# kaleo996/F5E-TTS

Measured on AMD Instinct MI355X. Metric: mel_frames_per_sec, higher is better.
Workload: dtype bf16; 1 GPU; C2: F5TTS_v1_Base random-init, batch 1 per GPU, N_ref=188 N=469 frames, euler NFE=32, CFG=2.0 (cond+uncond batched), sway=-1.0, hipGraph ODE loop, HIP log-mel front-end + Vocos decode on GPU; parallelism=replica x1 (utterance sharding, no collective on the data path)

## Files before the change

f5e-tts_amd/_C.py:

```python
from __future__ import annotations

import ctypes as C
import os

_HERE = os.path.dirname(os.path.abspath(__file__))
LIB_PATH = os.environ.get("F5E_HIP_LIB") or os.path.join(_HERE, "libf5e_hip.so")

ABI_VERSION = 2

ACT_NONE, ACT_SILU, ACT_GELU_ERF, ACT_GELU_TANH, ACT_RELU, ACT_MISH = range(6)

_P, _I, _F, _LL = C.c_void_p, C.c_int, C.c_float, C.c_longlong

SIGNATURES = {
    "f5e_abi_version": [],
    "f5e_last_error": [],
    "f5e_check_device": [],
    "f5e_gemm_bf16_bias": [_P, _P, _I, _P, _I, _P, _P, _I, _I, _I, _I, _I, _I, _I],
    "f5e_gemm_bf16_gate_residual": [_P, _P, _I, _P, _I, _P, _P, _I, _P, _I, _I, _P, _I, _I, _P, _I, _I, _I, _I],
    "f5e_gemm_bf16_qkv_rope": [_P, _P, _I, _P, _I, _P, _P, _P, _P, _I, _I, _I, _P, _P, _P, _I, _I, _I, _I],
    "f5e_gemm_bf16_bias_ln": [_P, _P, _I, _P, _I, _P, _P, _I, _I, _I, _I, _I, _I, _I, _P],
    "f5e_gemm_bf16_gate_residual_ln": [_P, _P, _I, _P, _I, _P, _P, _I, _P, _I, _I, _P, _I, _I, _P, _I, _I, _I, _I, _P],
    "f5e_gemm_bf16_qkv_rope_ln": [_P, _P, _I, _P, _I, _P, _P, _P, _P, _I, _I, _I, _P, _P, _P, _I, _I, _I, _I, _P],
    "f5e_adaln_pre": [_P, _P, _I, _P, _I, _P, _I, _I, _I, _P, _I, _P, _I, _P, _I, _I],
    "f5e_flash_attn": [_P, _P, _P, _P, _P, _I, _P, _I, _I, _I, _I, _I],
    "f5e_joint_attn": [_P, _P, _P, _P, _P, _P, _P, _P, _I, _P, _I, _P, _I, _I, _I, _I, _I, _I, _I],
    "f5e_layernorm": [_P, _P, _I, _P, _I, _I, _P, _P, _P, _P, _I, _I, _I, _P, _I, _I, _I, _F],
    "f5e_grn": [_P, _P, _P, _P, _P, _P, _I, _I, _I],
    "f5e_l2norm": [_P, _P, _I, _P, _I, _I, _P, _I, _I],
    "f5e_gemm_f32": [_P, _P, _I, _I, _I, _P, _I, _P, _I, _P, _P, _I, _I, _P, _P, _I, _P, _I, _I, _I, _I],
    "f5e_convpos": [_P, _P, _I, _P, _P, _I, _P, _I, _P, _I, _P, _I, _I, _I, _I, _I],
    "f5e_dwconv7": [_P, _P, _P, _P, _P, _I, _I, _I],
    "f5e_im2col": [_P, _P, _P, _I, _I, _I, _I, _I],
    "f5e_conv2d_sub_f32": [_P, _P, _P, _P, _P, _I, _I, _I, _I, _I, _I, _I, _I],
    "f5e_sinus_embed": [_P, _P, _P, _P, _I, _I, _F],
    "f5e_rope_table": [_P, _P, _P, _I, _I],
    "f5e_text_gather": [_P, _P, _P, _P, _P, _P, _I, _I, _I, _I, _I],
    "f5e_ode_update": [_P, _P, _LL, _I, _F, _F, _P, _P, _P, _P, _P, _P, _LL],
    "f5e_ode_update_traj": [_P, _P, _LL, _I, _F, _F, _P, _P, _P, _LL, _I, _P, _P, _P, _LL],
    "f5e_advance_eval": [_P, _P],
    "f5e_stitch": [_P, _P, _P, _P, _P, _LL, _I],
    "f5e_cast_bf16": [_P, _P, _P, _LL],
    "f5e_cast_f32": [_P, _P, _P, _LL],
    "f5e_axpby": [_P, _P, _P, _P, _F, _F, _F, _LL],
    "f5e_vq_eval": [_P, _P, _I, _P, _I, _P, _P, _P, _I, _I, _I, _I],
    "f5e_mas_workspace_bytes": [_I, _I, _I, C.POINTER(C.c_ulonglong)],
    "f5e_mas_path": [_P, _P, _LL, _I, _P, _P, _P, _P, _P, C.c_ulonglong, _I, _I, _I],
    "f5e_resample": [_P, _P, _LL, _P, _I, _I, _I, _P, _LL, _I, _I, _I],
    "f5e_ctc_align_workspace_bytes": [_I, _I, _I, C.POINTER(C.c_ulonglong)],
    "f5e_ctc_align": [_P, _P, _LL, _I, _P, _I, _P, _P, _I, _P, _P, _P, _P, _P, C.c_ulonglong, _I, _I, _I, _I],
    "f5e_ctc_greedy": [_P, _P, _LL, _I, _P, _I, _I, _P, _P, _P, _I, _I, _I],
    "f5e_ctc_loss_workspace_bytes": [_I, _I, C.POINTER(C.c_ulonglong)],
# ... 131 lines not shown
```

f5e-tts_amd/csrc/elementwise.hip:

```cpp
#include "f5e_common.h"

namespace {

inline int grid_for(size_t total) {
  size_t g = (total + 255) / 256;
  return (int)(g < 2048 ? (g ? g : 1) : 2048);
}

__global__ void sinus_embed_kernel(const float* t, const float* freqs, float* out, int E, int dim, float scale) {
  const int half = dim / 2;
  const int i = blockIdx.x * blockDim.x + threadIdx.x;
  if (i >= E * half) return;
  const int e = i / half, k = i - e * half;
  const float arg = (scale * t[e]) * freqs[k];
  float s, c;
  sincosf(arg, &s, &c);
  out[(size_t)e * dim + k] = s;
  out[(size_t)e * dim + half + k] = c;
}

__global__ void rope_table_kernel(const float* inv_freq, float* out, int N, int half) {
  const int i = blockIdx.x * blockDim.x + threadIdx.x;
  if (i >= N * half) return;
  const int n = i / half, k = i - n * half;
// ... 6 lines not shown

__global__ void text_gather_kernel(const int* ids, const float* table, const float* pos, const float* keep, float* out,
                                   int B, int N, int TD, int max_pos, int table_rows) {
  const int td4 = TD / 4;
  const size_t total = (size_t)B * N * td4;
  for (size_t i = (size_t)blockIdx.x * 256 + threadIdx.x; i < total; i += (size_t)gridDim.x * 256) {
    const int c = (int)(i % td4) * 4;
    const size_t bn = i / td4;
    const int n = (int)(bn % N);
    const int id = min(max(ids[bn], 0), table_rows - 1);
    f32x4 v = *(const f32x4*)(table + (size_t)id * TD + c);
    if (pos) v += *(const f32x4*)(pos + (size_t)min(n, max_pos - 1) * TD + c);
    if (keep) v *= keep[bn];
    *(f32x4*)(out + bn * TD + c) = v;
  }
}

__global__ void ode_update_kernel(const float* pred, size_t branch_stride, int mode, float w0, float w1,
                                  const float* base, float* dst, float* traj, size_t traj_stride, int traj_div,
                                  const float* coef, int* eval_ptr, unsigned* done_ctr, size_t n) {
  const int e = eval_ptr ? load_uniform_i32(eval_ptr) : 0;
  const float h = __builtin_bit_cast(float, load_uniform_i32((const int*)(coef + e)));
  if (traj && traj_stride) traj += (size_t)((e + 1) / traj_div) * traj_stride;
  for (size_t i = (size_t)blockIdx.x * 256 + threadIdx.x; i < n; i += (size_t)gridDim.x * 256) {
    const float p0 = pred[i];
    float v = p0;
    if (mode == 1) {
      v = p0 + (p0 - pred[i + branch_stride]) * w0;
    } else if (mode == 2) {
      const float p1 = pred[i + branch_stride], p2 = pred[i + 2 * branch_stride];
// ... 122 lines not shown
  const int total = N * half;
  hipLaunchKernelGGL(rope_table_kernel, dim3((total + 255) / 256), dim3(256), 0, st, inv_freq, out, N, half);
  F5E_LAUNCH_CHECK("rope_table");
  return F5E_OK;
}

int f5e_text_gather(hipStream_t st, const int* ids, const float* table, const float* pos, const float* keep,
                    float* out, int B, int N, int TD, int max_pos, int table_rows) {
  F5E_REQUIRE(ids && table && out && B > 0 && N > 0 && TD > 0 && TD % 4 == 0 && table_rows > 0, "text_gather: bad arguments");
  hipLaunchKernelGGL(text_gather_kernel, dim3(grid_for((size_t)B * N * TD / 4)), dim3(256), 0, st, ids, table, pos,
                     keep, out, B, N, TD, max_pos, table_rows);
  F5E_LAUNCH_CHECK("text_gather");
  return F5E_OK;
}

int f5e_ode_update(hipStream_t st, const float* pred, long long branch_stride, int mode, float w0, float w1,
                   const float* base, float* dst, float* traj, const float* coef, int* eval_ptr, unsigned* done_ctr,
                   long long n) {
  return f5e_ode_update_traj(st, pred, branch_stride, mode, w0, w1, base, dst, traj, 0, 1, coef, eval_ptr, done_ctr, n);
}

int f5e_ode_update_traj(hipStream_t st, const float* pred, long long branch_stride, int mode, float w0, float w1,
                        const float* base, float* dst, float* traj, long long traj_stride, int traj_div,
                        const float* coef, int* eval_ptr, unsigned* done_ctr, long long n) {
  F5E_REQUIRE(pred && base && dst && coef && n > 0, "ode_update: bad arguments");
  F5E_REQUIRE(mode >= 0 && mode <= 2, "ode_update: mode must be 0 (plain), 1 (cfg) or 2 (three-branch)");
  F5E_REQUIRE(!done_ctr || eval_ptr, "ode_update: done_ctr (auto-advance) needs eval_ptr");
  F5E_REQUIRE(traj_stride >= 0 && traj_div >= 1 && (traj_stride == 0 || eval_ptr), "ode_update: bad trajectory indexing");
  hipLaunchKernelGGL(ode_update_kernel, dim3(grid_for((size_t)n)), dim3(256), 0, st, pred, (size_t)branch_stride, mode,
                     w0, w1, base, dst, traj, (size_t)traj_stride, traj_div, coef, eval_ptr, done_ctr, (size_t)n);
// ... 60 lines not shown
```

f5e-tts_amd/csrc/gemm_f32.hip:

```cpp
#include "f5e_common.h"

namespace {

struct Gemm32Args {
  const float* A; int lda; int a_rows; int a_act;
  const float* W; int ldw;
  const float* bias;
  int act;
  const float* ch_scale;
  const float* addend; int ld_add; int add_rows;
  const float* row_scale;
  float* out; int ldo;
  bf16* out_bf16; int ldo_bf16;
  int M, N, K;
  int tiles_m;
  int vec;
};

__global__ __launch_bounds__(256) void gemm_f32_kernel(Gemm32Args a) {
  constexpr int BK = 16, LDS_ROW = 17;
  __shared__ float As[2][64 * LDS_ROW];
  __shared__ float Ws[2][64 * LDS_ROW];
  const int tid = threadIdx.x, lane = tid & 63, wave = tid >> 6;
  const int tile_n = blockIdx.x / a.tiles_m, tile_m = blockIdx.x - tile_n * a.tiles_m;
// ... 267 lines not shown
                            int add_rows, const float* row_scale, float* out, int ldo, void* out_bf16, int ldo_bf16,
                            int M, int N, int K) {
  F5E_REQUIRE(A && W && (out || out_bf16), "gemm_f32: null operand");
  F5E_REQUIRE(M > 0 && N > 0 && K > 0, "gemm_f32: empty problem M=%d N=%d K=%d", M, N, K);
  F5E_REQUIRE(K % 4 == 0 && lda % 4 == 0 && ldw % 4 == 0, "gemm_f32: K, lda, ldw must be multiples of 4 (K=%d)", K);
  F5E_REQUIRE(a_rows > 0, "gemm_f32: a_rows must be positive");
  if (addend) F5E_REQUIRE(add_rows > 0, "gemm_f32: add_rows must be positive");
  Gemm32Args a{};
  a.A = A; a.lda = lda; a.a_rows = a_rows; a.a_act = a_act; a.W = W; a.ldw = ldw; a.bias = bias; a.act = act;
  a.ch_scale = ch_scale; a.addend = addend; a.ld_add = ld_add; a.add_rows = add_rows > 0 ? add_rows : 1;
  a.row_scale = row_scale; a.out = out; a.ldo = ldo; a.out_bf16 = (bf16*)out_bf16; a.ldo_bf16 = ldo_bf16;
  a.M = M; a.N = N; a.K = K;
  a.vec = N % 4 == 0 && N >= 4 && ldo % 4 == 0 && ldo_bf16 % 4 == 0 && ld_add % 4 == 0 &&
          (((uintptr_t)bias | (uintptr_t)ch_scale | (uintptr_t)addend | (uintptr_t)out) & 15) == 0 && ((uintptr_t)out_bf16 & 7) == 0;
  if (a_act == F5E_ACT_NONE && (((uintptr_t)A | (uintptr_t)W) & 15) == 0) {
    if (((M + 63) / 64) * ((N + 63) / 64) < 128) return launch_dma<32, 64, 2, 2, 4>(a, st);
    return launch_dma<64, 64, 2, 2, 3>(a, st);
  }
  a.tiles_m = (M + 63) / 64;
  const int grid = a.tiles_m * ((N + 63) / 64);
  hipLaunchKernelGGL(gemm_f32_kernel, dim3(grid), dim3(256), 0, st, a);
  F5E_LAUNCH_CHECK("gemm_f32");
  return F5E_OK;
}
```

f5e-tts_amd/csrc/norm.hip:

```cpp
#include "f5e_common.h"

namespace {

struct LnArgs {
  const float* x; int ldx;
  void* y; int ldy; int y_bf16;
  const float* gamma; const float* beta;
  const float* scale; const float* shift;
  int mod_stride, mod_rows, rows_per_seq;
  int rows, D;
  float eps;
  const int* eval_ptr; int eval_stride;
};

template <int VPL>
__global__ __launch_bounds__(256) void layernorm_kernel(LnArgs a) {
  const int lane = threadIdx.x & 63;
  const int row = blockIdx.x * 4 + (threadIdx.x >> 6);
  if (row >= a.rows) return;
  const float* xp = a.x + (size_t)row * a.ldx;
  f32x4 v[VPL];
#pragma unroll
  for (int i = 0; i < VPL; ++i) v[i] = *(const f32x4*)(xp + (i * 64 + lane) * 4);
  const int mrow = a.scale ? (row / a.rows_per_seq) % a.mod_rows : 0;
// ... 50 lines not shown
#pragma unroll
  for (int i = 0; i < 8; ++i)
    if (i * 64 + lane < nv) {
      v[i] -= mean;
      ss += (v[i][0] * v[i][0] + v[i][1] * v[i][1]) + (v[i][2] * v[i][2] + v[i][3] * v[i][3]);
    }
  const float rstd = rsqrtf(wave_sum(ss) / (float)a.D + a.eps);
#pragma unroll
  for (int i = 0; i < 8; ++i) {
    const int c = (i * 64 + lane) * 4;
    if (c < a.D) {
      f32x4 y = v[i] * rstd;
      if (a.gamma) y = y * *(const f32x4*)(a.gamma + c) + *(const f32x4*)(a.beta + c);
      *(f32x4*)((float*)a.y + (size_t)row * a.ldy + c) = y;
    }
  }
}

template <int VPL>
__global__ __launch_bounds__(256) void adaln_pre_kernel(const float* x, int ldx, bf16* xs, int ld_xs, const float* scale,
                                                        int mod_stride, int mod_rows, int rows_per_seq,
                                                        const int* eval_ptr, int eval_stride, float* stats, int parts,
                                                        float* row_mean, int rows, int D) {
  const int lane = threadIdx.x & 63;
  const int row = blockIdx.x * 4 + (threadIdx.x >> 6);
  if (row >= rows) return;
  const float* xp = x + (size_t)row * ldx;
  f32x4 v[VPL], sc[VPL];
#pragma unroll
  for (int i = 0; i < VPL; ++i) v[i] = *(const f32x4*)(xp + (i * 64 + lane) * 4);
// ... 154 lines not shown
  F5E_REQUIRE(D % 256 == 0 && D >= 256 && D <= 2048, "layernorm: D=%d must be a multiple of 256 in [256, 2048]", D);
  switch (D / 256) {
    case 1: hipLaunchKernelGGL(layernorm_kernel<1>, grid, block, 0, st, a); break;
    case 2: hipLaunchKernelGGL(layernorm_kernel<2>, grid, block, 0, st, a); break;
    case 3: hipLaunchKernelGGL(layernorm_kernel<3>, grid, block, 0, st, a); break;
    case 4: hipLaunchKernelGGL(layernorm_kernel<4>, grid, block, 0, st, a); break;
    case 5: hipLaunchKernelGGL(layernorm_kernel<5>, grid, block, 0, st, a); break;
    case 6: hipLaunchKernelGGL(layernorm_kernel<6>, grid, block, 0, st, a); break;
    case 7: hipLaunchKernelGGL(layernorm_kernel<7>, grid, block, 0, st, a); break;
    default: hipLaunchKernelGGL(layernorm_kernel<8>, grid, block, 0, st, a); break;
  }
  F5E_LAUNCH_CHECK("layernorm");
  return F5E_OK;
}

int f5e_adaln_pre(hipStream_t st, const float* x, int ldx, void* xs, int ld_xs, const float* scale, int mod_stride,
                  int mod_rows, int rows_per_seq, const int* eval_ptr, int eval_stride, float* stats, int parts,
                  float* row_mean, int rows, int D) {
  F5E_REQUIRE(x && xs && scale && stats && row_mean && rows > 0, "adaln_pre: null/empty");
  F5E_REQUIRE(D % 256 == 0 && D >= 256 && D <= 2048, "adaln_pre: D=%d must be a multiple of 256 in [256, 2048]", D);
  F5E_REQUIRE(ldx % 4 == 0 && ld_xs % 4 == 0 && mod_stride % 4 == 0, "adaln_pre: strides must be multiples of 4");
  F5E_REQUIRE(parts > 0 && parts <= 32 && mod_rows > 0 && rows_per_seq > 0, "adaln_pre: bad parts / modulation rows");
  const dim3 grid((rows + 3) / 4), block(256);
#define F5E_PRE_CASE(V)                                                                                               \
  case V: hipLaunchKernelGGL(adaln_pre_kernel<V>, grid, block, 0, st, x, ldx, (bf16*)xs, ld_xs, scale, mod_stride,    \
                             mod_rows, rows_per_seq, eval_ptr, eval_stride, stats, parts, row_mean, rows, D); break;
  switch (D / 256) {
    F5E_PRE_CASE(1) F5E_PRE_CASE(2) F5E_PRE_CASE(3) F5E_PRE_CASE(4) F5E_PRE_CASE(5) F5E_PRE_CASE(6) F5E_PRE_CASE(7)
    default: hipLaunchKernelGGL(adaln_pre_kernel<8>, grid, block, 0, st, x, ldx, (bf16*)xs, ld_xs, scale, mod_stride,
                                mod_rows, rows_per_seq, eval_ptr, eval_stride, stats, parts, row_mean, rows, D); break;
// ... 42 lines not shown
```

f5e-tts_amd/engine.py:

```python
from __future__ import annotations

import math
import os
import threading
from dataclasses import dataclass
from typing import Dict, List, Optional, Tuple

import torch

from . import _C, ops

Tensor = torch.Tensor
BF, F32, I32 = torch.bfloat16, torch.float32, torch.int32


@dataclass
class DiTConfig:
    dim: int = 1024
    depth: int = 22
    heads: int = 16
    dim_head: int = 64
    ff_mult: int = 2
    mel_dim: int = 100
    text_num_embeds: int = 2545
# ... 234 lines not shown
        temb = self.time_embed(t2.reshape(-1))
        mod = torch.empty(E * rows, self.row_stride, device=dv)
        D = cfg.dim
        for l, (w, b) in enumerate(self.adaln):
            ops.gemm_f32(temb, w, b, out=mod[:, l * 6 * D:(l + 1) * 6 * D], a_act=ops.ACT_SILU)
        ops.gemm_f32(temb, self.final_w, self.final_b, out=mod[:, self.L * 6 * D:], a_act=ops.ACT_SILU)
        self._last_temb = temb
        return mod.view(E, rows, self.row_stride)

    def text_embed(self, text: Optional[Tensor], B: int, N: int, drop_text: bool) -> Tensor:
        return self.text_embed_multi(text, B, N, (drop_text,))[0]

    def text_embed_multi(self, text: Optional[Tensor], B: int, N: int, drops: Tuple[bool, ...]) -> List[Tensor]:
        cfg, dv = self.cfg, self.device
        V = len(drops)
        keep = None
        if text is None:
            ids = torch.zeros(V * B, N, dtype=I32, device=dv)
        else:
            if text.device.type == "cpu" and text[:, :N].numel():
                hi, lo = int(text[:, :N].max()), int(text[:, :N].min())
                if hi + 1 >= self.text_table.shape[0] or lo < -1:
                    raise IndexError(f"index out of range in self: token id {hi if hi + 1 >= self.text_table.shape[0] else lo} "
                                     f"with text_num_embeds = {self.text_table.shape[0] - 1}")
            ids = (h2d(text, dv) + 1)[:, :N]
            ids = torch.nn.functional.pad(ids, (0, N - ids.shape[1]), value=0)
            if cfg.text_mask_padding:
                keep = (ids != 0).to(F32).repeat(V, 1).contiguous()
            ids = torch.cat([torch.zeros_like(ids) if d else ids for d in drops], 0).to(I32).contiguous()
        TD = cfg.text_dim
        VB = V * B
        h = torch.empty(VB, N, TD, device=dv)
        ops.text_gather(ids, self.text_table, self.text_pos, keep if self.text_blocks else None, h)
        if self.text_blocks:
            c = torch.empty_like(h)
            n = torch.empty_like(h)
            p1 = torch.empty(VB, N, 2 * TD, device=dv)
            g = torch.empty_like(p1)
            gws = torch.empty(VB, 2 * TD, device=dv)
            keep_flat = keep.view(-1) if keep is not None else None
            for blk in self.text_blocks:
                ops.dwconv7(h, blk["dw_w"], blk["dw_b"], c)
                ops.layernorm(c.view(VB * N, TD), n.view(VB * N, TD), gamma=blk["ln_g"], beta=blk["ln_b"])
                ops.gemm_f32(n.view(VB * N, TD), blk["w1"], blk["b1"], out=p1.view(VB * N, 2 * TD), act=ops.ACT_GELU_ERF)
                ops.grn(p1, g, blk["grn_g"], blk["grn_b"], gws)
                h_new = torch.empty_like(h)
                ops.gemm_f32(g.view(VB * N, 2 * TD), blk["w2"], blk["b2"], out=h_new.view(VB * N, TD),
                             addend=h.view(VB * N, TD), row_scale=keep_flat)
                h = h_new
        return [h[v * B:(v + 1) * B] for v in range(V)]

    def ppg_embed(self, ppg: Optional[Tensor], B: int, N: int, drop_ppg: bool) -> Tensor:
        cfg, dv, P = self.cfg, self.device, self.ppg
        pd = cfg.ppg_dim
        x = torch.zeros(B, N, pd, device=dv)
        if ppg is not None and not drop_ppg:
            x[:, : ppg.shape[1]] = ppg.to(dv, F32)[:, :N]
        if cfg.ppg_transformer:
# ... 371 lines not shown
    cache: Dict[tuple, Tensor] = {}
    drops = tuple(sorted({dt_ for _, dt_, _ in inp.branches}))
    for dt_, emb in zip(drops, engine.text_embed_multi(inp.text, B, N, drops)):
        cache[("t", dt_)] = emb
    for bi, (da, dt_, dp) in enumerate(inp.branches):
        tk = ("t", dt_)
        pe = None
        if cfg.use_ppg:
            pk = ("p", dp)
            if pk not in cache:
                cache[pk] = engine.ppg_embed(inp.ppg, B, N, dp)
            pe = cache[pk]
        engine.input_const(inp.step_cond, cache[tk], pe, da, in_const[bi * B * N:(bi + 1) * B * N])
    if masked:
        seq_len.copy_(setup["seq_len"].repeat(nb))
    bf["ctr"].zero_()
    y.copy_(inp.y0)
    traj[0].copy_(inp.y0)

    if fresh:
        def plans_for(y_in, first_ws):
            out = []
            for c in range(n_chains):
                lo, hi = c * per * B * N, (c + 1) * per * B * N
                sl = seq_len[c * per * B:(c + 1) * per * B] if seq_len is not None else None
                out.append(engine.make_plan(per * B, B, N, y_in, in_const[lo:hi], mod, eval_ptr, rope_cs, sl,
                                            pred=pred_all[lo:hi], cd=cd, arena=bf["ws"][first_ws + c]))
            return out

        st.plans_a = plans_for(y, 0)
        st.plans_b = plans_for(y_mid, n_chains) if y_mid is not None else None
    if st.pool is None or st.pool.owner is not st:
        for pl in st.plans_a + (st.plans_b or []):
# ... 97 lines not shown
```

f5e-tts_amd/model/cfm.py:

```python
from __future__ import annotations

from typing import Callable, NamedTuple, Optional

import torch
import torch.nn.functional as F
from torch import nn

from .. import _C
from ..engine import SamplerInputs, h2d, ode_setup, run_ode
from .modules import MelSpec
from .utils import default, exists, intersperse, lens_to_mask, list_str_to_idx, list_str_to_tensor

F32, I32 = torch.float32, torch.int32


class Alignment(NamedTuple):
    token_of_frame: torch.Tensor
    durations: torch.Tensor
    text_len: torch.Tensor
    ppg_len: torch.Tensor


class CFM(nn.Module):
    def __init__(self, transformer: nn.Module, sigma=0.0, odeint_kwargs: dict = dict(method="euler"),
                 audio_drop_prob=0.3, cond_drop_prob=0.2, num_channels=None, mel_spec_module: nn.Module | None = None,
                 mel_spec_kwargs: dict = dict(), frac_lengths_mask: tuple[float, float] = (0.7, 1.0),
                 vocab_char_map: dict[str, int] | None = None, ppg_config=dict(use_ppg=False),
                 cb_config=dict(use_codebook=False)):
        super().__init__()
        self.frac_lengths_mask = frac_lengths_mask
        self.mel_spec = default(mel_spec_module, MelSpec(**mel_spec_kwargs))
        self.num_channels = default(num_channels, self.mel_spec.n_mel_channels)
        self.audio_drop_prob, self.cond_drop_prob = audio_drop_prob, cond_drop_prob
        self.transformer = transformer
        self.dim = transformer.dim
# ... 56 lines not shown
        else:
            dur_h = torch.maximum(lens_h + 1, dur_h)
        dur_h = dur_h.clamp(max=max_duration)
        n = int(dur_h.amax())
        test_cond = None
        if duplicate_test:
            test_cond = F.pad(cond, (0, 0, cond_seq_len, n - 2 * cond_seq_len), value=0.0)
        cond = F.pad(cond, (0, 0, 0, n - cond_seq_len), value=0.0)
        if no_ref_audio:
            cond = torch.zeros_like(cond)
        if edit_mask is not None:
            cond_mask = h2d(cond_mask, dv) & edit_mask.to(dv)
        cond_mask = h2d(F.pad(cond_mask, (0, n - cond_mask.shape[-1]), value=False), dv).unsqueeze(-1)
        from .. import ops
        cond = cond.contiguous()
        step_cond = ops.stitch(cond, torch.zeros_like(cond), cond_mask.reshape(-1).to(torch.uint8).contiguous(),
                               torch.empty_like(cond))
        seq_len = dur_h.to(I32) if batch > 1 else None
        y0 = torch.zeros(batch, n, self.num_channels, dtype=F32)
        for i, dur in enumerate(dur_h.tolist()):
            if exists(seed):
                gen = torch.Generator().manual_seed(seed)
                y0[i, :dur] = torch.randn(dur, self.num_channels, dtype=F32, generator=gen)
            else:
                y0[i, :dur] = torch.randn(dur, self.num_channels, dtype=F32)
        y0 = h2d(y0, dv)
        t_start = 0
        if duplicate_test:
            t_start = t_inter
            y0 = ops.axpby(y0, test_cond.contiguous(), torch.empty_like(y0), 1 - t_start, t_start)
            steps = int(steps * (1 - t_start))
# ... 6 lines not shown
        eng = self.transformer.engine()
        inp = SamplerInputs(step_cond=prep["step_cond"], text=prep["text"], ppg=ppg, y0=prep["y0"], t=prep["t"],
                            seq_len=prep["seq_len"], branches=branches, mode=mode, w0=w0, w1=w1,
                            method=self.odeint_kwargs.get("method", "euler"))
        if self.use_graph:
            side = getattr(self._tls, "stream", None)
            if side is None:
                side = self._tls.stream = torch.cuda.Stream(device=eng.device)
            setup = ode_setup(eng, inp)
            trajectory = run_ode(eng, inp, use_graph=True, chains=self.chains, setup=setup, capture_stream=side)
        else:
            trajectory = run_ode(eng, inp, use_graph=False, timer=self.kernel_timer, chains=self.chains)
        self.transformer.clear_cache()
        out = torch.empty_like(trajectory[-1])
        from .. import ops
        ops.stitch(prep["cond"].contiguous(), trajectory[-1], prep["cond_mask"].reshape(-1).to(torch.uint8).contiguous(),
                   out)
        if exists(vocoder):
            out = vocoder(out.permute(0, 2, 1))
        return out, trajectory


    @torch.no_grad()
    def sample(self, cond, text, ppg=None, duration=None, *, lens=None, steps=32, cfg_strength=1.0,
               sway_sampling_coef=None, seed: Optional[int] = None, max_duration=4096,
               vocoder: Optional[Callable] = None, no_ref_audio=False, duplicate_test=False, t_inter=0.1,
               edit_mask=None):
        prep = self._prepare(cond, text, duration, lens, steps, sway_sampling_coef, seed, max_duration, no_ref_audio,
                             duplicate_test, t_inter, edit_mask, use_text=True)
        if cfg_strength < 1e-5:
            return self._integrate(prep, ppg, [(False, False, False)], 0, 0.0, 0.0, vocoder)
# ... 55 lines not shown
```

f5e-tts_amd/ops.py:

```python
from __future__ import annotations

import ctypes as C
import threading
from typing import Optional

import torch

from . import _C
from ._C import ACT_GELU_ERF, ACT_GELU_TANH, ACT_MISH, ACT_NONE, ACT_RELU, ACT_SILU, check, lib

Tensor = torch.Tensor
_checked_device = False


def _stream() -> int:
    return torch.cuda.current_stream().cuda_stream


def require_device() -> None:
    global _checked_device
    if not _checked_device:
        if not torch.cuda.is_available():
            raise _C.F5EError("f5e_tts_amd needs a ROCm GPU (gfx950); torch.cuda.is_available() is False and there "
                              "is no CPU fallback")
# ... 246 lines not shown
                            mode, _p(out_bf16, BF, "out_bf16"), out_bf16.stride(0) if out_bf16 is not None else 0,
                            _p(out_f32, F32, "out_f32"), out_f32.stride(0) if out_f32 is not None else 0,
                            _p(resid, F32, "resid"), resid.stride(0) if resid is not None else 0, S, N, D,
                            w_packed.shape[0]),
          "f5e_convpos")


def dwconv7(x: Tensor, w_t: Tensor, bias: Tensor, out: Tensor):
    require_device()
    B, T, Cc = x.shape
    check(lib().f5e_dwconv7(_stream(), _p(x, F32, "x"), _p(w_t, F32, "w_t"), _p(bias, F32, "bias"), _p(out, F32, "out"),
                            B, T, Cc), "f5e_dwconv7")
    return out


def im2col(x: Tensor, col: Tensor, ksize: int, pad: int):
    require_device()
    B, T, Cin = x.shape
    check(lib().f5e_im2col(_stream(), _p(x, F32, "x"), _p(col, F32, "col"), B, T, Cin, ksize, pad), "f5e_im2col")
    return col


def pack_conv2d_sub_weight(w: Tensor) -> Tensor:
    return w.permute(0, 2, 3, 1).contiguous()


def conv2d_sub(x: Tensor, w_packed: Tensor, bias: Optional[Tensor], stride: int, *, out: Optional[Tensor] = None,
               act: int = ACT_RELU) -> Tensor:
    require_device()
    if x.ndim != 4 or w_packed.ndim != 4:
# ... 26 lines not shown

def rope_table(inv_freq: Tensor, out: Tensor):
    require_device()
    N, half, _ = out.shape
    check(lib().f5e_rope_table(_stream(), _p(inv_freq, F32, "inv_freq"), _p(out, F32, "out"), N, half), "f5e_rope_table")
    return out


def text_gather(ids: Tensor, table: Tensor, pos: Optional[Tensor], keep: Optional[Tensor], out: Tensor):
    require_device()
    B, N, TD = out.shape
    check(lib().f5e_text_gather(_stream(), _p(ids, I32, "ids"), _p(table, F32, "table"), _p(pos, F32, "pos"),
                                _p(keep, F32, "keep"), _p(out, F32, "out"), B, N, TD,
                                pos.shape[0] if pos is not None else 1, table.shape[0]), "f5e_text_gather")
    return out


def ode_update(pred: Tensor, branch_stride: int, mode: int, w0: float, w1: float, base: Tensor, dst: Tensor,
               coef: Tensor, eval_ptr: Optional[Tensor], traj: Optional[Tensor] = None,
               done_ctr: Optional[Tensor] = None, traj_stride: int = 0, traj_div: int = 1):
    require_device()
    check(lib().f5e_ode_update_traj(_stream(), _p(pred, F32, "pred"), branch_stride, mode, w0, w1, _p(base, F32, "base"),
                                    _p(dst, F32, "dst"), C.c_void_p(traj.data_ptr()) if traj is not None else None,
                                    traj_stride, traj_div, _p(coef, F32, "coef"), _p(eval_ptr, I32, "eval_ptr"),
                                    _p(done_ctr, I32, "done_ctr"), base.numel()), "f5e_ode_update")
    return dst


def sample_loop(loop: "_C.LoopPlan"):
    require_device()
# ... 974 lines not shown
```

f5e-tts_amd/vocoder.py:

```python
from __future__ import annotations

import os
from typing import Optional

import torch
from torch import nn

from . import _C, ops
from .engine import fft_tables

F32 = torch.float32


class _ConvNeXtBlock(nn.Module):
    def __init__(self, dim, intermediate_dim, layer_scale_init_value):
        super().__init__()
        self.dwconv = nn.Conv1d(dim, dim, kernel_size=7, padding=3, groups=dim)
        self.norm = nn.LayerNorm(dim, eps=1e-6)
        self.pwconv1 = nn.Linear(dim, intermediate_dim)
        self.act = nn.GELU()
        self.pwconv2 = nn.Linear(intermediate_dim, dim)
        self.gamma = nn.Parameter(layer_scale_init_value * torch.ones(dim))


# ... 69 lines not shown
            raise _C.F5EError("Vocos.decode expects [b, n_mels, t]")
        dv = mel.device
        w = self._pack(dv)
        B, Cin, T = mel.shape
        if T < 2:
            raise _C.F5EError("Vocos.decode needs at least 2 frames")
        x = mel.to(F32).transpose(1, 2).contiguous()
        dim = w["embed_b"].shape[0]
        col = torch.empty(B, T, 7 * Cin, device=dv)
        ops.im2col(x, col, 7, 3)
        h = torch.empty(B * T, dim, device=dv)
        ops.gemm_f32(col.view(B * T, 7 * Cin), w["embed_w"], w["embed_b"], out=h)
        hn = torch.empty_like(h)
        ops.layernorm(h, hn, gamma=w["norm_g"], beta=w["norm_b"])
        h = hn
        c = torch.empty_like(h)
        n = torch.empty_like(h)
        inter = w["blocks"][0]["w1"].shape[0] if w["blocks"] else dim
        p1 = torch.empty(B * T, inter, device=dv)
        for blk in w["blocks"]:
            ops.dwconv7(h.view(B, T, dim), blk["dw_w"], blk["dw_b"], c.view(B, T, dim))
            ops.layernorm(c, n, gamma=blk["ln_g"], beta=blk["ln_b"])
            ops.gemm_f32(n, blk["w1"], blk["b1"], out=p1, act=ops.ACT_GELU_ERF)
            h_new = torch.empty_like(h)
            ops.gemm_f32(p1, blk["w2"], blk["b2"], out=h_new, ch_scale=blk["gamma"], addend=h)
            h = h_new
        ops.layernorm(h, n, gamma=w["fin_g"], beta=w["fin_b"])
        n_fft, hop = self.head.n_fft, self.head.hop_length
        z = torch.empty(B * T, n_fft + 2, device=dv)
        ops.gemm_f32(n, w["out_w"], w["out_b"], out=z)
        frames = torch.empty(B * T, n_fft, device=dv)
        wav = torch.empty(B, hop * (T - 1), device=dv)
        ops.istft_head(z, w["window"], w["twiddle"], frames, wav, B, T, n_fft, hop)
        return wav

    def forward(self, mel):
        return self.decode(mel)
# ... 11 lines not shown
```

include/f5e_abi.h:

```cpp
#ifndef F5E_ABI_H_
#define F5E_ABI_H_

#ifdef __cplusplus
extern "C" {
#endif

#define F5E_ABI_VERSION 2

#if defined(__GNUC__)
#define F5E_API __attribute__((visibility("default")))
#else
#define F5E_API
#endif

enum { F5E_OK = 0, F5E_ERR_BAD_SHAPE = -1, F5E_ERR_UNSUPPORTED = -2, F5E_ERR_HIP = -3 };

enum { F5E_ACT_NONE = 0, F5E_ACT_SILU = 1, F5E_ACT_GELU_ERF = 2, F5E_ACT_GELU_TANH = 3, F5E_ACT_RELU = 4, F5E_ACT_MISH = 5 };

#ifdef F5E_STREAM_T
typedef F5E_STREAM_T f5e_stream;
#else
typedef void* f5e_stream;
#endif

// ... 57 lines not shown
F5E_API int f5e_grn(f5e_stream st, const float* x, float* y, float* gx_ws, const float* gamma, const float* beta, int B, int T,
            int C);


F5E_API int f5e_gemm_f32(f5e_stream st, const float* A, int lda, int a_rows, int a_act, const float* W, int ldw,
                 const float* bias, int act, const float* ch_scale, const float* addend, int ld_add, int add_rows,
                 const float* row_scale, float* out, int ldo, void* out_bf16, int ldo_bf16, int M, int N, int K);


F5E_API int f5e_convpos(f5e_stream st, const void* x, int ldx, const void* w_packed, const float* bias, int mode,
                void* out_bf16, int ldo, float* out_f32, int ldo32, const float* resid, int ldr, int S, int N, int D,
                int groups);

F5E_API int f5e_dwconv7(f5e_stream st, const float* x, const float* w_t, const float* bias, float* y, int B, int T, int C);

F5E_API int f5e_im2col(f5e_stream st, const float* x, float* col, int B, int T, int Cin, int ksize, int pad);

F5E_API int f5e_conv2d_sub_f32(f5e_stream st, const float* x, const float* w, const float* bias, float* y, int B, int T_in,
                       int F_in, int C, int kt, int kf, int stride, int act);


F5E_API int f5e_sinus_embed(f5e_stream st, const float* t, const float* freqs, float* out, int E, int dim, float scale);
F5E_API int f5e_rope_table(f5e_stream st, const float* inv_freq, float* out, int N, int half);
F5E_API int f5e_text_gather(f5e_stream st, const int* ids, const float* table, const float* pos, const float* keep, float* out,
                    int B, int N, int TD, int max_pos, int table_rows);
F5E_API int f5e_ode_update(f5e_stream st, const float* pred, long long branch_stride, int mode, float w0, float w1,
                   const float* base, float* dst, float* traj, const float* coef, int* eval_ptr, unsigned* done_ctr,
                   long long n);
F5E_API int f5e_ode_update_traj(f5e_stream st, const float* pred, long long branch_stride, int mode, float w0, float w1,
                        const float* base, float* dst, float* traj, long long traj_stride, int traj_div,
                        const float* coef, int* eval_ptr, unsigned* done_ctr, long long n);
F5E_API int f5e_advance_eval(f5e_stream st, int* eval_ptr);
F5E_API int f5e_stitch(f5e_stream st, const float* cond, const float* y, const unsigned char* mask, float* out, long long rows,
               int C);
F5E_API int f5e_cast_bf16(f5e_stream st, const float* x, void* y, long long n);
F5E_API int f5e_cast_f32(f5e_stream st, const void* x, float* y, long long n);
F5E_API int f5e_axpby(f5e_stream st, const float* x, const float* y, float* out, float a, float b, float c, long long n);
F5E_API int f5e_vq_eval(f5e_stream st, const float* logits, int ld, const float* vars, int combine_groups, float* out,
                int* targets, float* stats, int rows, int groups, int num_vars, int var_dim);

// ... 233 lines not shown
```

Before: 12750 mel-frames/s.

## Fuse dwconv7+layernorm, fuse text id prep and ODE init, retune small-GEMM tile

Adds a fused depthwise conv7 + LayerNorm kernel used in the text ConvNeXt blocks and the Vocos blocks, which removes the intermediate buffer and one launch per block. Text-embedding id preparation (offset, pad, mask, CFG drop concat) moves into a single gather kernel that reads int64 token ids directly, replacing several small torch ops. ODE state initialisation (counter zero plus two copies) becomes one kernel. The small-problem threshold in the f32 GEMM now uses 32x32 tiles, scaled by CU count. These mostly trim per-utterance launch overhead outside the graphed ODE loop, so their effect on throughput is likely small.

```diff
diff --git a/f5e-tts_amd/_C.py b/f5e-tts_amd/_C.py
--- a/f5e-tts_amd/_C.py
+++ b/f5e-tts_amd/_C.py
@@ -31,11 +31,14 @@
     "f5e_gemm_f32": [_P, _P, _I, _I, _I, _P, _I, _P, _I, _P, _P, _I, _I, _P, _P, _I, _P, _I, _I, _I, _I],
     "f5e_convpos": [_P, _P, _I, _P, _P, _I, _P, _I, _P, _I, _P, _I, _I, _I, _I, _I],
     "f5e_dwconv7": [_P, _P, _P, _P, _P, _I, _I, _I],
+    "f5e_dwconv7_ln": [_P, _P, _P, _P, _P, _P, _P, _I, _I, _I, _F],
     "f5e_im2col": [_P, _P, _P, _I, _I, _I, _I, _I],
     "f5e_conv2d_sub_f32": [_P, _P, _P, _P, _P, _I, _I, _I, _I, _I, _I, _I, _I],
     "f5e_sinus_embed": [_P, _P, _P, _P, _I, _I, _F],
     "f5e_rope_table": [_P, _P, _P, _I, _I],
     "f5e_text_gather": [_P, _P, _P, _P, _P, _P, _I, _I, _I, _I, _I],
+    "f5e_text_gather_ids": [_P, _P, _I, _I, C.c_uint, _P, _P, _P, _P, _I, _I, _I, _I, _I, _I],
+    "f5e_ode_init": [_P, _P, _P, _P, _P, _LL],
     "f5e_ode_update": [_P, _P, _LL, _I, _F, _F, _P, _P, _P, _P, _P, _P, _LL],
     "f5e_ode_update_traj": [_P, _P, _LL, _I, _F, _F, _P, _P, _P, _LL, _I, _P, _P, _P, _LL],
     "f5e_advance_eval": [_P, _P],
diff --git a/f5e-tts_amd/csrc/elementwise.hip b/f5e-tts_amd/csrc/elementwise.hip
--- a/f5e-tts_amd/csrc/elementwise.hip
+++ b/f5e-tts_amd/csrc/elementwise.hip
@@ -44,6 +44,39 @@
     if (keep) v *= keep[bn];
     *(f32x4*)(out + bn * TD + c) = v;
   }
+}
+
+__global__ void text_gather_ids_kernel(const long long* text, int ld_text, int nt, unsigned drop_bits, const float* table,
+                                       const float* pos, float* keep_out, float* out, int V, int B, int N, int TD,
+                                       int max_pos, int table_rows) {
+  const int td4 = TD / 4;
+  const size_t total = (size_t)V * B * N * td4;
+  for (size_t i = (size_t)blockIdx.x * 256 + threadIdx.x; i < total; i += (size_t)gridDim.x * 256) {
+    const int c4 = (int)(i % td4);
+    const size_t bn = i / td4;
+    const int n = (int)(bn % N);
+    const size_t vb = bn / N;
+    const int b = (int)(vb % B), v = (int)(vb / B);
+    const int raw = n < nt ? (int)(text[(size_t)b * ld_text + n] + 1) : 0;
+    const float k = raw != 0 ? 1.0f : 0.0f;
+    const int id = min(max((drop_bits >> v) & 1u ? 0 : raw, 0), table_rows - 1);
+    f32x4 val = *(const f32x4*)(table + (size_t)id * TD + c4 * 4);
+    if (pos) val += *(const f32x4*)(pos + (size_t)min(n, max_pos - 1) * TD + c4 * 4);
+    if (keep_out) {
+      val *= k;
+      if (c4 == 0) keep_out[bn] = k;
+    }
+    *(f32x4*)(out + bn * TD + c4 * 4) = val;
+  }
+}
+
+__global__ void ode_init_kernel(const float* y0, float* y, float* traj0, int* ctr, size_t n) {
+  for (size_t i = (size_t)blockIdx.x * 256 + threadIdx.x; i < n; i += (size_t)gridDim.x * 256) {
+    const float v = y0[i];
+    y[i] = v;
+    if (traj0) traj0[i] = v;
+  }
+  if (blockIdx.x == 0 && threadIdx.x < 2) ctr[threadIdx.x] = 0;
 }
 
 __global__ void ode_update_kernel(const float* pred, size_t branch_stride, int mode, float w0, float w1,
@@ -196,6 +229,25 @@
   return F5E_OK;
 }
 
+int f5e_text_gather_ids(hipStream_t st, const long long* text, int ld_text, int nt, unsigned drop_bits, const float* table,
+                        const float* pos, float* keep_out, float* out, int V, int B, int N, int TD, int max_pos,
+                        int table_rows) {
+  F5E_REQUIRE(text && table && out && V > 0 && V <= 32 && B > 0 && N > 0 && TD > 0 && TD % 4 == 0 && table_rows > 0,
+              "text_gather_ids: bad arguments");
+  F5E_REQUIRE(nt >= 0 && nt <= N && ld_text >= nt, "text_gather_ids: nt=%d columns of a row of %d, N=%d", nt, ld_text, N);
+  hipLaunchKernelGGL(text_gather_ids_kernel, dim3(grid_for((size_t)V * B * N * TD / 4)), dim3(256), 0, st, text, ld_text, nt,
+                     drop_bits, table, pos, keep_out, out, V, B, N, TD, max_pos, table_rows);
+  F5E_LAUNCH_CHECK("text_gather_ids");
+  return F5E_OK;
+}
+
+int f5e_ode_init(hipStream_t st, const float* y0, float* y, float* traj0, int* ctr, long long n) {
+  F5E_REQUIRE(y0 && y && ctr && n > 0, "ode_init: bad arguments");
+  hipLaunchKernelGGL(ode_init_kernel, dim3(grid_for((size_t)n)), dim3(256), 0, st, y0, y, traj0, ctr, (size_t)n);
+  F5E_LAUNCH_CHECK("ode_init");
+  return F5E_OK;
+}
+
 int f5e_ode_update(hipStream_t st, const float* pred, long long branch_stride, int mode, float w0, float w1,
                    const float* base, float* dst, float* traj, const float* coef, int* eval_ptr, unsigned* done_ctr,
                    long long n) {
diff --git a/f5e-tts_amd/csrc/gemm_f32.hip b/f5e-tts_amd/csrc/gemm_f32.hip
--- a/f5e-tts_amd/csrc/gemm_f32.hip
+++ b/f5e-tts_amd/csrc/gemm_f32.hip
@@ -305,7 +305,7 @@
   a.vec = N % 4 == 0 && N >= 4 && ldo % 4 == 0 && ldo_bf16 % 4 == 0 && ld_add % 4 == 0 &&
           (((uintptr_t)bias | (uintptr_t)ch_scale | (uintptr_t)addend | (uintptr_t)out) & 15) == 0 && ((uintptr_t)out_bf16 & 7) == 0;
   if (a_act == F5E_ACT_NONE && (((uintptr_t)A | (uintptr_t)W) & 15) == 0) {
-    if (((M + 63) / 64) * ((N + 63) / 64) < 128) return launch_dma<32, 64, 2, 2, 4>(a, st);
+    if (((M + 31) / 32) * ((N + 31) / 32) <= 2 * f5e_cu_count()) return launch_dma<32, 32, 2, 2, 3>(a, st);
     return launch_dma<64, 64, 2, 2, 3>(a, st);
   }
   a.tiles_m = (M + 63) / 64;
diff --git a/f5e-tts_amd/csrc/norm.hip b/f5e-tts_amd/csrc/norm.hip
--- a/f5e-tts_amd/csrc/norm.hip
+++ b/f5e-tts_amd/csrc/norm.hip
@@ -88,6 +88,47 @@
       if (a.gamma) y = y * *(const f32x4*)(a.gamma + c) + *(const f32x4*)(a.beta + c);
       *(f32x4*)((float*)a.y + (size_t)row * a.ldy + c) = y;
     }
+  }
+}
+
+template <int VPL>
+__global__ __launch_bounds__(256) void dwconv7_ln_kernel(const float* x, const float* wT, const float* bias,
+                                                          const float* gamma, const float* beta, float* y, int rows,
+                                                          int T, int D, float eps) {
+  const int lane = threadIdx.x & 63;
+  const int row = blockIdx.x * 4 + (threadIdx.x >> 6);
+  if (row >= rows) return;
+  const int t = row % T;
+  f32x4 v[VPL];
+#pragma unroll
+  for (int i = 0; i < VPL; ++i) {
+    const int c = (i * 64 + lane) * 4;
+    f32x4 acc = *(const f32x4*)(bias + c);
+#pragma unroll
+    for (int j = 0; j < 7; ++j) {
+      const int tj = t + j - 3;
+      if (tj >= 0 && tj < T)
+        acc += *(const f32x4*)(wT + (size_t)j * D + c) * *(const f32x4*)(x + ((size_t)row + j - 3) * D + c);
+    }
+    v[i] = acc;
+  }
+  float s = 0.f;
+#pragma unroll
+  for (int i = 0; i < VPL; ++i) s += (v[i][0] + v[i][1]) + (v[i][2] + v[i][3]);
+  const float mean = wave_sum(s) / (float)D;
+  float ss = 0.f;
+#pragma unroll
+  for (int i = 0; i < VPL; ++i) {
+    v[i] -= mean;
+    ss += (v[i][0] * v[i][0] + v[i][1] * v[i][1]) + (v[i][2] * v[i][2] + v[i][3] * v[i][3]);
+  }
+  const float rstd = rsqrtf(wave_sum(ss) / (float)D + eps);
+#pragma unroll
+  for (int i = 0; i < VPL; ++i) {
+    const int c = (i * 64 + lane) * 4;
+    f32x4 o = v[i] * rstd;
+    o = o * *(const f32x4*)(gamma + c) + *(const f32x4*)(beta + c);
+    *(f32x4*)(y + (size_t)row * D + c) = o;
   }
 }
 
@@ -272,6 +313,29 @@
   return F5E_OK;
 }
 
+int f5e_dwconv7_ln(hipStream_t st, const float* x, const float* w_t, const float* bias, const float* gamma,
+                   const float* beta, float* y, int B, int T, int C, float eps) {
+  F5E_REQUIRE(x && w_t && bias && gamma && beta && y, "dwconv7_ln: null operand");
+  F5E_REQUIRE(x != y, "dwconv7_ln: y must not be x (rows read their neighbours)");
+  F5E_REQUIRE(B > 0 && T > 0 && C > 0 && C % 4 == 0, "dwconv7_ln: C=%d must be a positive multiple of 4", C);
+  const long long rows = (long long)B * T;
+  F5E_REQUIRE(rows <= 0x7fffffff, "dwconv7_ln: B * T = %lld rows do not fit an int", rows);
+  if (C % 256 != 0 || C > 1024) {
+    const int rc = f5e_dwconv7(st, x, w_t, bias, y, B, T, C);
+    if (rc != F5E_OK) return rc;
+    return f5e_layernorm(st, y, C, y, C, 0, gamma, beta, nullptr, nullptr, 0, 0, 1, nullptr, 0, (int)rows, C, eps);
+  }
+  const dim3 grid((unsigned)((rows + 3) / 4)), block(256);
+  switch (C / 256) {
+    case 1: hipLaunchKernelGGL(dwconv7_ln_kernel<1>, grid, block, 0, st, x, w_t, bias, gamma, beta, y, (int)rows, T, C, eps); break;
+    case 2: hipLaunchKernelGGL(dwconv7_ln_kernel<2>, grid, block, 0, st, x, w_t, bias, gamma, beta, y, (int)rows, T, C, eps); break;
+    case 3: hipLaunchKernelGGL(dwconv7_ln_kernel<3>, grid, block, 0, st, x, w_t, bias, gamma, beta, y, (int)rows, T, C, eps); break;
+    default: hipLaunchKernelGGL(dwconv7_ln_kernel<4>, grid, block, 0, st, x, w_t, bias, gamma, beta, y, (int)rows, T, C, eps); break;
+  }
+  F5E_LAUNCH_CHECK("dwconv7_ln");
+  return F5E_OK;
+}
+
 int f5e_adaln_pre(hipStream_t st, const float* x, int ldx, void* xs, int ld_xs, const float* scale, int mod_stride,
                   int mod_rows, int rows_per_seq, const int* eval_ptr, int eval_stride, float* stats, int parts,
                   float* row_mean, int rows, int D) {
diff --git a/f5e-tts_amd/engine.py b/f5e-tts_amd/engine.py
--- a/f5e-tts_amd/engine.py
+++ b/f5e-tts_amd/engine.py
@@ -272,34 +272,37 @@
     def text_embed_multi(self, text: Optional[Tensor], B: int, N: int, drops: Tuple[bool, ...]) -> List[Tensor]:
         cfg, dv = self.cfg, self.device
         V = len(drops)
-        keep = None
-        if text is None:
-            ids = torch.zeros(V * B, N, dtype=I32, device=dv)
-        else:
-            if text.device.type == "cpu" and text[:, :N].numel():
-                hi, lo = int(text[:, :N].max()), int(text[:, :N].min())
-                if hi + 1 >= self.text_table.shape[0] or lo < -1:
-                    raise IndexError(f"index out of range in self: token id {hi if hi + 1 >= self.text_table.shape[0] else lo} "
-                                     f"with text_num_embeds = {self.text_table.shape[0] - 1}")
-            ids = (h2d(text, dv) + 1)[:, :N]
-            ids = torch.nn.functional.pad(ids, (0, N - ids.shape[1]), value=0)
-            if cfg.text_mask_padding:
-                keep = (ids != 0).to(F32).repeat(V, 1).contiguous()
-            ids = torch.cat([torch.zeros_like(ids) if d else ids for d in drops], 0).to(I32).contiguous()
         TD = cfg.text_dim
         VB = V * B
         h = torch.empty(VB, N, TD, device=dv)
-        ops.text_gather(ids, self.text_table, self.text_pos, keep if self.text_blocks else None, h)
+        keep = None
+        if text is not None and text.device.type == "cpu" and text[:, :N].numel():
+            hi, lo = int(text[:, :N].max()), int(text[:, :N].min())
+            if hi + 1 >= self.text_table.shape[0] or lo < -1:
+                raise IndexError(f"index out of range in self: token id {hi if hi + 1 >= self.text_table.shape[0] else lo} "
+                                 f"with text_num_embeds = {self.text_table.shape[0] - 1}")
+        if text is None or text.numel() == 0 or text.ndim != 2 or text.shape[0] != B or V > 32:
+            if text is None:
+                ids = torch.zeros(VB, N, dtype=I32, device=dv)
+            else:
+                ids = (h2d(text, dv) + 1)[:, :N]
+                ids = torch.nn.functional.pad(ids, (0, N - ids.shape[1]), value=0)
+                if cfg.text_mask_padding:
+                    keep = (ids != 0).to(F32).repeat(V, 1).contiguous()
+                ids = torch.cat([torch.zeros_like(ids) if d else ids for d in drops], 0).to(I32).contiguous()
+            ops.text_gather(ids, self.text_table, self.text_pos, keep if self.text_blocks else None, h)
+        else:
+            if cfg.text_mask_padding and self.text_blocks:
+                keep = torch.empty(VB, N, device=dv)
+            ops.text_gather_ids(h2d(text, dv, torch.int64), drops, self.text_table, self.text_pos, keep, h)
         if self.text_blocks:
-            c = torch.empty_like(h)
             n = torch.empty_like(h)
             p1 = torch.empty(VB, N, 2 * TD, device=dv)
             g = torch.empty_like(p1)
             gws = torch.empty(VB, 2 * TD, device=dv)
             keep_flat = keep.view(-1) if keep is not None else None
             for blk in self.text_blocks:
-                ops.dwconv7(h, blk["dw_w"], blk["dw_b"], c)
-                ops.layernorm(c.view(VB * N, TD), n.view(VB * N, TD), gamma=blk["ln_g"], beta=blk["ln_b"])
+                ops.dwconv7_ln(h, blk["dw_w"], blk["dw_b"], blk["ln_g"], blk["ln_b"], n)
                 ops.gemm_f32(n.view(VB * N, TD), blk["w1"], blk["b1"], out=p1.view(VB * N, 2 * TD), act=ops.ACT_GELU_ERF)
                 ops.grn(p1, g, blk["grn_g"], blk["grn_b"], gws)
                 h_new = torch.empty_like(h)
@@ -701,9 +704,7 @@
         engine.input_const(inp.step_cond, cache[tk], pe, da, in_const[bi * B * N:(bi + 1) * B * N])
     if masked:
         seq_len.copy_(setup["seq_len"].repeat(nb))
-    bf["ctr"].zero_()
-    y.copy_(inp.y0)
-    traj[0].copy_(inp.y0)
+    ops.ode_init(inp.y0.to(dv, F32).contiguous(), y, traj[0], bf["ctr"])
 
     if fresh:
         def plans_for(y_in, first_ws):
diff --git a/f5e-tts_amd/model/cfm.py b/f5e-tts_amd/model/cfm.py
--- a/f5e-tts_amd/model/cfm.py
+++ b/f5e-tts_amd/model/cfm.py
@@ -19,6 +19,11 @@
     durations: torch.Tensor
     text_len: torch.Tensor
     ppg_len: torch.Tensor
+
+
+def _mask_bytes(mask: torch.Tensor) -> torch.Tensor:
+    mask = mask.reshape(-1).contiguous()
+    return mask.view(torch.uint8) if mask.dtype == torch.bool else mask.to(torch.uint8)
 
 
 class CFM(nn.Module):
@@ -105,7 +110,7 @@
         cond_mask = h2d(F.pad(cond_mask, (0, n - cond_mask.shape[-1]), value=False), dv).unsqueeze(-1)
         from .. import ops
         cond = cond.contiguous()
-        step_cond = ops.stitch(cond, torch.zeros_like(cond), cond_mask.reshape(-1).to(torch.uint8).contiguous(),
+        step_cond = ops.stitch(cond, torch.zeros_like(cond), _mask_bytes(cond_mask),
                                torch.empty_like(cond))
         seq_len = dur_h.to(I32) if batch > 1 else None
         y0 = torch.zeros(batch, n, self.num_channels, dtype=F32)
@@ -142,7 +147,7 @@
         self.transformer.clear_cache()
         out = torch.empty_like(trajectory[-1])
         from .. import ops
-        ops.stitch(prep["cond"].contiguous(), trajectory[-1], prep["cond_mask"].reshape(-1).to(torch.uint8).contiguous(),
+        ops.stitch(prep["cond"].contiguous(), trajectory[-1], _mask_bytes(prep["cond_mask"]),
                    out)
         if exists(vocoder):
             out = vocoder(out.permute(0, 2, 1))
diff --git a/f5e-tts_amd/ops.py b/f5e-tts_amd/ops.py
--- a/f5e-tts_amd/ops.py
+++ b/f5e-tts_amd/ops.py
@@ -284,6 +284,19 @@
     return out
 
 
+def dwconv7_ln(x: Tensor, w_t: Tensor, bias: Tensor, gamma: Tensor, beta: Tensor, out: Tensor, eps: float = 1e-6):
+    require_device()
+    if x.ndim != 3 or out.shape != x.shape or not x.is_contiguous() or not out.is_contiguous():
+        raise _C.F5EError(f"dwconv7_ln: x and out must be contiguous [B, T, C] of one shape (got {tuple(x.shape)}, {tuple(out.shape)})")
+    B, T, Cc = x.shape
+    if w_t.shape != (7, Cc) or not w_t.is_contiguous() or bias.numel() != Cc or gamma.numel() != Cc or beta.numel() != Cc:
+        raise _C.F5EError(f"dwconv7_ln: w_t must be contiguous [7, {Cc}], bias / gamma / beta [{Cc}]")
+    check(lib().f5e_dwconv7_ln(_stream(), _p(x, F32, "x"), _p(w_t, F32, "w_t"), _p(bias, F32, "bias"),
+                               _p(gamma, F32, "gamma"), _p(beta, F32, "beta"), _p(out, F32, "out"), B, T, Cc, float(eps)),
+          "f5e_dwconv7_ln")
+    return out
+
+
 def im2col(x: Tensor, col: Tensor, ksize: int, pad: int):
     require_device()
     B, T, Cin = x.shape
@@ -340,6 +353,34 @@
                                 _p(keep, F32, "keep"), _p(out, F32, "out"), B, N, TD,
                                 pos.shape[0] if pos is not None else 1, table.shape[0]), "f5e_text_gather")
     return out
+
+
+def text_gather_ids(text: Tensor, drops, table: Tensor, pos: Optional[Tensor], keep_out: Optional[Tensor], out: Tensor):
+    require_device()
+    VB, N, TD = out.shape
+    V = len(drops)
+    if text.ndim != 2 or text.dtype != torch.int64 or not text.is_cuda or (text.shape[1] > 1 and text.stride(1) != 1):
+        raise _C.F5EError("text_gather_ids: text must be an int64 GPU tensor [B, nt] with unit column stride")
+    B = text.shape[0]
+    if V < 1 or V > 32 or VB != V * B or not out.is_contiguous() or (keep_out is not None and keep_out.numel() != VB * N):
+        raise _C.F5EError(f"text_gather_ids: out must be contiguous [{V} * {B}, N, TD], keep_out [{V} * {B}, N]")
+    bits = sum(1 << v for v, d in enumerate(drops) if d)
+    check(lib().f5e_text_gather_ids(_stream(), C.c_void_p(text.data_ptr()), text.stride(0), min(text.shape[1], N), bits,
+                                    _p(table, F32, "table"), _p(pos, F32, "pos"), _p(keep_out, F32, "keep_out"),
+                                    _p(out, F32, "out"), V, B, N, TD, pos.shape[0] if pos is not None else 1,
+                                    table.shape[0]), "f5e_text_gather_ids")
+    return out
+
+
+def ode_init(y0: Tensor, y: Tensor, traj0: Optional[Tensor], ctr: Tensor):
+    require_device()
+    for t in (y0, y) + ((traj0,) if traj0 is not None else ()):
+        if not t.is_contiguous() or t.numel() != y0.numel():
+            raise _C.F5EError("ode_init: y0, y and traj0 must be contiguous and of one size")
+    if ctr.numel() != 2 or not ctr.is_contiguous():
+        raise _C.F5EError("ode_init: ctr must be int32[2]")
+    check(lib().f5e_ode_init(_stream(), _p(y0, F32, "y0"), _p(y, F32, "y"), _p(traj0, F32, "traj0"), _p(ctr, I32, "ctr"),
+                             y0.numel()), "f5e_ode_init")
 
 
 def ode_update(pred: Tensor, branch_stride: int, mode: int, w0: float, w1: float, base: Tensor, dst: Tensor,
diff --git a/f5e-tts_amd/vocoder.py b/f5e-tts_amd/vocoder.py
--- a/f5e-tts_amd/vocoder.py
+++ b/f5e-tts_amd/vocoder.py
@@ -107,13 +107,11 @@
         hn = torch.empty_like(h)
         ops.layernorm(h, hn, gamma=w["norm_g"], beta=w["norm_b"])
         h = hn
-        c = torch.empty_like(h)
         n = torch.empty_like(h)
         inter = w["blocks"][0]["w1"].shape[0] if w["blocks"] else dim
         p1 = torch.empty(B * T, inter, device=dv)
         for blk in w["blocks"]:
-            ops.dwconv7(h.view(B, T, dim), blk["dw_w"], blk["dw_b"], c.view(B, T, dim))
-            ops.layernorm(c, n, gamma=blk["ln_g"], beta=blk["ln_b"])
+            ops.dwconv7_ln(h.view(B, T, dim), blk["dw_w"], blk["dw_b"], blk["ln_g"], blk["ln_b"], n.view(B, T, dim))
             ops.gemm_f32(n, blk["w1"], blk["b1"], out=p1, act=ops.ACT_GELU_ERF)
             h_new = torch.empty_like(h)
             ops.gemm_f32(p1, blk["w2"], blk["b2"], out=h_new, ch_scale=blk["gamma"], addend=h)
diff --git a/include/f5e_abi.h b/include/f5e_abi.h
--- a/include/f5e_abi.h
+++ b/include/f5e_abi.h
@@ -95,6 +95,9 @@
 
 F5E_API int f5e_dwconv7(f5e_stream st, const float* x, const float* w_t, const float* bias, float* y, int B, int T, int C);
 
+F5E_API int f5e_dwconv7_ln(f5e_stream st, const float* x, const float* w_t, const float* bias, const float* gamma,
+                   const float* beta, float* y, int B, int T, int C, float eps);
+
 F5E_API int f5e_im2col(f5e_stream st, const float* x, float* col, int B, int T, int Cin, int ksize, int pad);
 
 F5E_API int f5e_conv2d_sub_f32(f5e_stream st, const float* x, const float* w, const float* bias, float* y, int B, int T_in,
@@ -105,6 +108,10 @@
 F5E_API int f5e_rope_table(f5e_stream st, const float* inv_freq, float* out, int N, int half);
 F5E_API int f5e_text_gather(f5e_stream st, const int* ids, const float* table, const float* pos, const float* keep, float* out,
                     int B, int N, int TD, int max_pos, int table_rows);
+F5E_API int f5e_text_gather_ids(f5e_stream st, const long long* text, int ld_text, int nt, unsigned drop_bits,
+                        const float* table, const float* pos, float* keep_out, float* out, int V, int B, int N, int TD,
+                        int max_pos, int table_rows);
+F5E_API int f5e_ode_init(f5e_stream st, const float* y0, float* y, float* traj0, int* ctr, long long n);
 F5E_API int f5e_ode_update(f5e_stream st, const float* pred, long long branch_stride, int mode, float w0, float w1,
                    const float* base, float* dst, float* traj, const float* coef, int* eval_ptr, unsigned* done_ctr,
                    long long n);
```

Measured after the change: 12810 mel-frames/s (median of 6 runs). About the same (+0.5%).
